# klkuhlm/unconfined

Measured on AMD Instinct MI355X. Metric: (t,r) drawdown points/sec, Neuman-1974 1024x256 sweep; max |rel err| vs CPU ref, higher is better.
Workload: dtype f64

## Files before the change

unconfined_amd/csrc/ucf_device.h:

```cpp

#include "ucf_math.h"
#include "ucf_plan.h"
#include <type_traits>

namespace UCF_NS {

using namespace ucfm;

#define UCF_STR_(x) #x
#define UCF_STR(x) UCF_STR_(x)
#define UCF_PI 3.14159265358979323846
#define UCF_EPS 2.220446049250313e-16

UCF_DEV double shfl_down1(double v) { return __shfl_down(v, 1, 64); }
UCF_DEV double shift_down1(double x)
{
    const int lo = __double2loint(x), hi = __double2hiint(x);
    const int l2 = __builtin_amdgcn_update_dpp(lo, lo, 0x130, 0xf, 0xf, false);
    const int h2 = __builtin_amdgcn_update_dpp(hi, hi, 0x130, 0xf, 0xf, false);
    return __hiloint2double(h2, l2);
}
UCF_DEV cplx shfl_down1(cplx v) { return cmake(shift_down1(v.re), shift_down1(v.im)); }
UCF_DEV cplx bcast0(cplx v) { return cmake(__shfl(v.re, 0, 64), __shfl(v.im, 0, 64)); }
UCF_DEV double wave_max(double v)
{
#pragma unroll
    for (int off = 32; off >= 1; off >>= 1) v = fmax(v, __shfl_xor(v, off, 64));
    return v;
}
UCF_DEV void stat_add(long long* ctr, bool pred)
{
    if (ctr == nullptr) return;
    unsigned long long bal = __ballot(pred);
    if (bal != 0ull && (threadIdx.x & 63) == 0) atomicAdd((unsigned long long*)ctr, (unsigned long long)__popcll(bal));
}

#ifndef UCF_TU
#define UCF_TU -1
#endif
#define UCF_TU_HAS(L) (UCF_TU < 0 || UCF_TU == (L))

typedef double2 lds_c;
UCF_DEV cplx lds_ld(const lds_c* base, int slot, int lane) { lds_c v = base[slot * UCF_WAVE + lane]; return cmake(v.x, v.y); }
UCF_DEV void lds_st(lds_c* base, int slot, int lane, cplx z) { base[slot * UCF_WAVE + lane] = make_double2(z.re, z.im); }
template <int PART = UCF_PART>
UCF_DEV cplx scr_ld(const lds_c* base, int slot, int lane) { lds_c v = base[slot * PART + (lane & (PART - 1))]; return cmake(v.x, v.y); }
template <int PART = UCF_PART>
UCF_DEV void scr_st(lds_c* base, int slot, int lane, cplx z) { base[slot * PART + (lane & (PART - 1))] = make_double2(z.re, z.im); }

#if UCF_FAST
UCF_DEV cplx cinv_plain_(cplx z)
{
    const double r = fast_rcp(z.re * z.re + z.im * z.im);
    return cmake(z.re * r, -(z.im * r));
}
#endif

UCF_DEV cplx lap_time(const ucf_dev_params& P, cplx p)
{
    if (P.timeType < 0) {
        const bool linear = P.timeType <= -101;
        const int n = linear ? -P.timeType - 100 : -P.timeType;
        cplx sum = cmake(0.0, 0.0);
        for (int k = 0; k < n; k++) {
            const cplx term = rscale(P.sched[n + k], cexp_(rscale(-P.sched[k], p)));
            sum = (k == 0) ? term : cadd(sum, term);
        }
        const cplx num = csub(sum, rscale(P.sched[2 * n + 1], cexp_(rscale(-P.sched[2 * n], p))));
        return cdiv(num, linear ? cmul(p, p) : p);
    }
    const double t1 = P.timePar[0], t2 = P.timePar[1];
    switch (P.timeType) {
    case 1: return cdiv(cexp_(cscale(p, -t1)), p);
    case 2: return csub(cdiv(cexp_(cscale(p, -t1)), p), cdiv(cexp_(cscale(p, -t2)), p));
    case 3: return cexp_(cscale(p, -t1));
    case 4: {
        cplx a = rdiv(1.0, csub(p, cmul(p, cexp_(cscale(p, -t1)))));
        cplx b = rsub(1.0, cexp_(cscale(p, -t2)));
        return cdiv(cmul(a, b), p);
    }
    case 5: return cdiv(cexp_(cscale(p, -t2)), cadd(p, cmul(p, cexp_(cscale(p, -t1)))));
    case 6: return cdiv(cmul(cexp_(cscale(p, -t2)), p), caddr(cmul(p, p), t1 * t1));
    case 7: return cmake(0.0, 0.0);
    case 8: {
        cplx ex = cexp_(cdivr(cscale(p, -t1), 2.0));
        cplx num = cmul(cexp_(cscale(p, -t2)), rsub(1.0, ex));
        return cdiv(num, cmul(radd(1.0, ex), p));
    }
    default: return cmake(__builtin_nan(""), __builtin_nan(""));
    }
}

struct k01 { cplx k0, k1; int ierr; };
UCF_DEV cplx clog_(cplx z) { return cmake(log(hypot(z.re, z.im)), atan2(z.im, z.re)); }

__device__ __noinline__ static k01 cbesk01_(cplx z)
{
    k01 out;
    out.k0 = cmake(0.0, 0.0); out.k1 = out.k0; out.ierr = 0;
    const double tol = UCF_EPS;
    const double elim = 2.303 * (1021.0 * log10(2.0) - 3.0);
    const double alim = elim + fmax(-(log10(2.0) * 52.0 * 2.303), -41.45);
    const double at1 = 0.78539816339744830962;
    const double pi = 4.0 * at1, hpi = 2.0 * at1, spi = 3.0 / (2.0 * at1);
    const double rthpi = sqrt(8.0 * at1) / 2.0, fpi = 1.89769999331517738, tth = 6.66666666666666666e-01;
    const double gamma_e = 5.77215664901532861e-01;
    const double xx = z.re, yy = z.im;
    if (xx == 0.0 && yy == 0.0) { out.ierr = 1; return out; }
    const double caz = hypot(xx, yy);
    if (caz > 1073741823.5) { out.ierr = 4; return out; }
    if (caz < UCF_DBL_MIN * 1.0e3) { out.ierr = 2; return out; }
    if (!(caz > tol) && -log(0.5 * caz) > elim) { out.ierr = 2; return out; }
    const cplx rz = cdiv(cmake(2.0, 0.0), z);
    cplx s1, s2;
    if (caz <= 2.0) {
        const cplx smu = clog_(rz);
        cplx f = cadd(rscale(-gamma_e, cmake(1.0, 0.0)), cscale(smu, 1.0));
        cplx p = cmake(0.5, 0.0), q = cmake(0.5, 0.0);
        s1 = f; s2 = p;
        double ak = 1.0, a1 = 1.0, bk = 1.0;
        cplx ck = cmake(1.0, 0.0);
        if (caz >= tol) {
            const cplx cz = cscale(cmul(z, z), 0.25);
            const double t1 = 0.25 * caz * caz;
            do {
// ... 1371 lines not shown
    const ucf_dev_params& P = P0;
    UCF_K1_ASSUME
#endif
    const int lane = threadIdx.x & (UCF_WAVE - 1), wv = __builtin_amdgcn_readfirstlane(threadIdx.x / UCF_WAVE);
    constexpr int EF = (FAMILY == 5) ? 1 : FAMILY;
    constexpr bool ZPAIR = FOLD && EF == 2 && NZC == 1;
    const int nz = NZC ? NZC : P0.nz, R = P0.R, nacc = P0.nacc, N = P0.N, ngl = P0.ngl;
    __builtin_assume(nz >= 1 && R >= 1 && nacc >= 1 && ngl >= 1);
    const int nabs = N + nacc * ngl;
    {
        const double2* __restrict__ gt = (const double2*)P0.sc_tab;
        for (int k = threadIdx.x; k < UCF_SC_ENTRIES; k += UCF_WAVE * UCF_IWPB) lds[k] = gt[k];
    }
    __syncthreads();
    const lds_c* sct = lds;
    const int lslots = (NZC ? R : R + 1) * nz;
    lds_c* const wlds = lds + UCF_SC_ENTRIES + (size_t)wv * lslots * UCF_WAVE;
    lds_c* accTS = wlds;
    lds_c* accCur = wlds + (size_t)R * nz * UCF_WAVE;
    int ustat = blockIdx.x * UCF_IWPB + wv - gridDim.x * UCF_IWPB;
    auto next_unit = [&]() {
        if (!wcount) return ustat += gridDim.x * UCF_IWPB;
        int u = 0;
        if (lane == 0) u = __hip_atomic_fetch_add(wcount, 1, __ATOMIC_RELAXED, __HIP_MEMORY_SCOPE_AGENT);
        return __builtin_amdgcn_readfirstlane(u);
    };
    for (int wi = next_unit(); wi < nworkw; wi = next_unit()) {
        const bool tail = wi >= nheadw;
        const int ls = tail ? (lsplit >> 8) : (lsplit & 255), nsplit = 1 << ls;
        const int wj = tail ? wi - nheadw : wi;
        const int pt = (tail ? (nheadw >> (lsplit & 255)) : 0) + (wj >> ls), sub = wj & (nsplit - 1);
        auto part_bound = [&](int k) {
            if (k <= 0) return 0;
            if (k >= nsplit) return nabs;
            int j = (k * nabs / nsplit - N + ngl / 2) / ngl;
            j = j < 0 ? 0 : (j > nacc ? nacc : j);
            return N + j * ngl;
        };
        const int n0 = part_bound(sub), n1 = part_bound(sub + 1);
        if (n1 <= n0 && sub != 0) continue;
#ifdef UCF_TIMELINE
        const unsigned long long tl_t0 = __builtin_amdgcn_s_memtime();
#endif
        const work_item W = decode_item<LAYOUT>(P0, pt, lane, per_point, nr, nt, ir0, npts);
        const ucf_dev_params& P = item_params<MULTI>(P0, Pv, (LAYOUT == 3 ? W.plan * ppp : W.pidx) + pbase, ppp);
        bool need_lay1 = false, need_lay3 = false, need_lay12 = false;
        for (int z = 0; z < nz; z++) { need_lay1 |= (P.zLay[z] == 1); need_lay3 |= (P.zLay[z] == 3); need_lay12 |= (P.zLay[z] != 3); }
        const double tD = tDv[W.it], rD = rDv[W.ir];
        const int sv = (LAYOUT == 1) ? svmin : svv[W.it];
        const double2* __restrict__ row = tab + (size_t)(per_point ? W.pidx : (W.ir * nsv + (sv - svmin))) * nabs;
        const double tee = 2.0 * tD;
        const double sigma = P.alpha - P.logtol / (2.0 * tee);
        const cplx p = cmake(sigma, UCF_PI * W.mlap / tee);
        const double2 ltv = ltab[(size_t)(W.mlap < P0.np ? W.mlap : P0.np - 1) * nrows + W.it];
        const cplx lt = cmake(ltv.x, ltv.y);
        const lane_consts LC = make_lane_consts(P, p, lt);
        auto lt_again = [&]() {
            int it = W.it;
            asm volatile("" : "+v"(it));
            const double2 v = ltab[(size_t)(W.mlap < P0.np ? W.mlap : P0.np - 1) * nrows + it];
            return cmake(v.x, v.y);
        };
        double2* __restrict__ sti = state + (size_t)pt * state_slots(P0) * UCF_WAVE;
        double2* __restrict__ areas = sti + (size_t)(R + 1) * nz * UCF_WAVE;
        for (int s = 0; s < lslots; s++) lds_st(wlds, s, lane, cmake(0.0, 0.0));
        fast_common F;
        sc_ctx_init(F.sc, sct, UCF_KV(FAMILY, FOLD));
        const bool lane_ok = FAMILY != 2 || (fabs(LC.xifac.re) + fabs(LC.xifac.im) < 1.0e90);
        const int nlim = (__builtin_amdgcn_ballot_w64(!lane_ok) == 0) ? n1 : n0;

        int n = n0;
        double2 aa = row[n0 < nabs ? n0 : 0];
        int m = 0, jj = n0 > N ? (n0 - N) / ngl : 0;
        cplx acc0 = cmake(0.0, 0.0), acc1 = cmake(0.0, 0.0);
        int zph = 0;
        if constexpr (ZPAIR) {
            int stopped = 0;
            zph = 0;
            static_assert(!ZPAIR || (LAYOUT == 1 && !MULTI),
                          "the interval ends and the limits of the bounds stand behind the rows of a grid's abscissa table only");
            const double* __restrict__ ends = (const double*)tab + abscissa_ends_offset((size_t)nr * nsv, nabs) + (size_t)(W.ir * nsv + (sv - svmin)) * (nacc + 1);
            const double* __restrict__ zb = (const double*)tab + abscissa_limits_offset((size_t)nr * nsv, nabs, nacc);
            int settled = 0;
            if (nlim > n0) zph = zpair_part_phase(P, LC, ends[nlim > N ? (nlim - N + ngl - 1) / ngl : 0]);
            const int nts = nlim < N ? nlim : N;
            auto proven_run = [&](auto cls, auto beta, int nend) {
                for (; n < nend; n++) {
                    const double2 nxt = row[n + 1 < nabs ? n + 1 : n];
                    F.sc.salt = n;
                    (void)fast_eta<2, true>(P, LC, aa.x, F);
                    const cplx val = rscale(aa.y, fast_sample_zpair_proven<decltype(cls)::value, decltype(beta)::value>(P, LC, F));
                    const int n1 = n + 1;
                    int tz = __builtin_ctz(n1);
                    if (tz > R - 1) tz = R - 1;
                    for (int sh = 0; sh <= tz; sh++) {
                        const int j = R - sh;
                        const double wl = P.ts_w[(size_t)(j - 1) * N + ((n1 >> sh) - 1)];
                        lds_st(accTS, j - 1, lane, cadd(lds_ld(accTS, j - 1, lane), rscale(wl, val)));
                    }
                    aa = nxt;
                }
            };
            auto proven_run_class = [&](auto cls, int nend) {
                if (P.beta != 0.0) proven_run(cls, std::true_type(), nend);
                else proven_run(cls, std::false_type(), nend);
            };
            constexpr int TS_RUNS = 2;
            for (int k = 1; k <= TS_RUNS && n < nts; k++) {
                int nend = k * N / TS_RUNS;
                if (nend > nts) nend = nts;
                if (nend <= n) continue;
                int cls = UCF_IV_EX_SHORT;
                if (!settled) {
                    int known;
                    cls = zpair_interval_class(P, LC, n == 0 ? 0.0 : aa.x, row[nend - 1].x, P.zD[0], &known, zb);
                    zph |= known;
                    if (cls == UCF_IV_EX_SHORT && (zph & UCF_PH_RANGE)) settled = 1;
                }
                if (cls == UCF_IV_CS_TAB) proven_run_class(std::integral_constant<int, UCF_IV_CS_TAB>(), nend);
                else if (cls == UCF_IV_CS_SHORT) proven_run_class(std::integral_constant<int, UCF_IV_CS_SHORT>(), nend);
                else if (cls == UCF_IV_EX_TAB) proven_run_class(std::integral_constant<int, UCF_IV_EX_TAB>(), nend);
                else if (cls == UCF_IV_EX_SHORT) proven_run_class(std::integral_constant<int, UCF_IV_EX_SHORT>(), nend);
                else {
                    for (; n < nend; n++) {
                        const double2 nxt = row[n + 1 < nabs ? n + 1 : n];
                        F.sc.salt = n;
                        if (!fast_eta_wave_zpair(P, LC, aa.x, F, zph, 1)) { stopped = 1; break; }
                        const cplx val = rscale(aa.y, fast_sample_zpair(P, LC, F, zph, 1));
                        const int n1 = n + 1;
                        int tz = __builtin_ctz(n1);
                        if (tz > R - 1) tz = R - 1;
                        for (int sh = 0; sh <= tz; sh++) {
                            const int j = R - sh;
                            const double wl = P.ts_w[(size_t)(j - 1) * N + ((n1 >> sh) - 1)];
                            lds_st(accTS, j - 1, lane, cadd(lds_ld(accTS, j - 1, lane), rscale(wl, val)));
                        }
                        aa = nxt;
                    }
                    if (stopped) break;
                }
                UCF_UNIFORM_BLOCK();
            }
            auto proven_interval = [&](auto cls, auto beta) {
                for (int i = 0; i < ngl; i++, n++) {
                    const double2 nxt = row[n + 1 < nabs ? n + 1 : n];
                    F.sc.salt = n;
                    (void)fast_eta<2, true>(P, LC, aa.x, F);
                    const cplx fz = fast_sample_zpair_proven<decltype(cls)::value, decltype(beta)::value>(P, LC, F);
                    acc0 = cmake(__builtin_fma(fz.re, aa.y, acc0.re), __builtin_fma(fz.im, aa.y, acc0.im));
                    aa = nxt;
                }
            };
            auto proven_class = [&](auto cls) {
                if (P.beta != 0.0) proven_interval(cls, std::true_type());
                else proven_interval(cls, std::false_type());
            };
            double lob_next = 0.0;
            if (!stopped && n < nlim) lob_next = ends[jj];
            if (!stopped) while (n < nlim) {
                const double lob = lob_next;
                const double hib = lob_next = ends[jj + 1];
                int cls = UCF_IV_UNPROVEN;
                if (settled) cls = UCF_IV_EX_SHORT;
                else {
                    int known;
                    cls = zpair_interval_class(P, LC, lob, hib, P.zD[0], &known, zb);
                    zph |= known;
                    if (cls == UCF_IV_EX_SHORT && (zph & UCF_PH_RANGE)) settled = 1;
                }
                if (cls == UCF_IV_CS_TAB) proven_class(std::integral_constant<int, UCF_IV_CS_TAB>());
                else if (cls == UCF_IV_CS_SHORT) proven_class(std::integral_constant<int, UCF_IV_CS_SHORT>());
                else if (cls == UCF_IV_EX_TAB) proven_class(std::integral_constant<int, UCF_IV_EX_TAB>());
                else if (cls == UCF_IV_EX_SHORT) proven_class(std::integral_constant<int, UCF_IV_EX_SHORT>());
                else {
                    for (m = 0; m < ngl; m++, n++) {
                        const double2 nxt = row[n + 1 < nabs ? n + 1 : n];
                        F.sc.salt = n;
                        const int last = m == ngl - 1;
                        if (!fast_eta_wave_zpair(P, LC, aa.x, F, zph, last)) { stopped = 1; break; }
                        const cplx fz = fast_sample_zpair(P, LC, F, zph, last);
                        acc0 = cmake(__builtin_fma(fz.re, aa.y, acc0.re), __builtin_fma(fz.im, aa.y, acc0.im));
                        aa = nxt;
                    }
                    if (stopped) break;
                }
                UCF_UNIFORM_BLOCK();
                {
                    const double hw = (hib - lob) / 2.0;
                    const cplx ar = cmul(rscale(hw, acc0), lt_again());
                    areas[(size_t)jj * UCF_WAVE + lane] = make_double2(ar.re, ar.im);
                    acc0 = cmake(0.0, 0.0);
                    m = 0;
                    jj++;
                }
            }
        } else
        for (; n < nlim; n++) {
            const double2 nxt = row[n + 1 < nabs ? n + 1 : n];
            const bool ts = n < N;
            F.sc.salt = n;
            if (!fast_eta_wave<EF>(P, LC, aa.x, F)) break;
            fast_common_terms<EF, FOLD, LAY3, LAY1, NOFOLD>(P, LC, aa.x, need_lay1, F, need_lay3, need_lay12);
            const int n1 = n + 1;
            int tz = __builtin_ctz(n1);
            if (tz > R - 1) tz = R - 1;
            for (int z = 0; z < nz; z++) {
                const cplx fz = fast_sample_z<EF, FOLD, LAY3, LAY1, NOFOLD>(P, F, z);
                if (ts) {
                    const cplx val = rscale(aa.y, fz);
                    for (int sh = 0; sh <= tz; sh++) {
                        const int j = R - sh;
                        const double wl = P.ts_w[(size_t)(j - 1) * N + ((n1 >> sh) - 1)];
                        const int slot = (j - 1) * nz + z;
                        lds_st(accTS, slot, lane, cadd(lds_ld(accTS, slot, lane), rscale(wl, val)));
                    }
                } else if (nz == 1 || (NZC == 2 && z == 0)) {
                    acc0 = cmake(__builtin_fma(fz.re, aa.y, acc0.re), __builtin_fma(fz.im, aa.y, acc0.im));
                } else if (NZC == 2) {
                    acc1 = cmake(__builtin_fma(fz.re, aa.y, acc1.re), __builtin_fma(fz.im, aa.y, acc1.im));
                } else {
                    const cplx a1 = lds_ld(accCur, z, lane);
                    lds_st(accCur, z, lane, cmake(__builtin_fma(fz.re, aa.y, a1.re), __builtin_fma(fz.im, aa.y, a1.im)));
                }
            }
            if (!ts && ++m == ngl) {
                const double lob = P.j0z[sv + jj - 1] / rD;
                const double hib = P.j0z[sv + jj] / rD;
                const double hw = (hib - lob) / 2.0;
                for (int z = 0; z < nz; z++) {
                    const cplx run = (nz == 1 || (NZC == 2 && z == 0)) ? acc0 : (NZC == 2 ? acc1 : lds_ld(accCur, z, lane));
                    const cplx ar = cmul(rscale(hw, run), lt);
                    areas[(size_t)(jj * nz + z) * UCF_WAVE + lane] = make_double2(ar.re, ar.im);
                    if (nz != 1 && NZC != 2) lds_st(accCur, z, lane, cmake(0.0, 0.0));
                }
                acc0 = acc1 = cmake(0.0, 0.0);
                m = 0;
                jj++;
            }
            aa = nxt;
        }
        if (sub == 0) {
            const cplx lte = ZPAIR ? lt_again() : lt;
            for (int s = 0; s < R * nz; s++) {
                const cplx v = cmul(lds_ld(wlds, s, lane), lte);
                sti[(size_t)s * UCF_WAVE + lane] = make_double2(v.re, v.im);
            }
            for (int s = R * nz; s < (R + 1) * nz; s++) sti[(size_t)s * UCF_WAVE + lane] = make_double2(0.0, 0.0);
        }
#ifdef UCF_TIMELINE
        if (sub == 0) {
            const unsigned long long tl_t1 = __builtin_amdgcn_s_memtime();
            const unsigned hwid = __builtin_amdgcn_s_getreg(63492);
            if (lane == 0) sti[(size_t)(R * nz) * UCF_WAVE + 0] = make_double2(__longlong_as_double((long long)tl_t0), __longlong_as_double((long long)tl_t1));
            if (lane == 1) sti[(size_t)(R * nz) * UCF_WAVE + 1] = make_double2((double)hwid, (double)__builtin_amdgcn_s_getreg(63508));
// ... 476 lines not shown
```

unconfined_amd/csrc/ucf_fastpath.h:

```cpp
#pragma once

namespace UCF_NS {

#define UCF_UNIFORM_BLOCK() asm volatile("" ::: "memory")
#define UCF_UNIFORM_BLOCK_F(FAMILY) do { if constexpr ((FAMILY) != 4) UCF_UNIFORM_BLOCK(); } while (0)

struct fprim {
    double ch, sh, ei, sn, cs;
};

template <bool POS, bool SMALLY = false>
UCF_DEV fprim prim_from_e(double x, double ax, double e, double ei, double y, const sc_ctx& sc)
{
    const int salt = sc.salt;
    fprim f;
    f.ei = ei;
    const double he = 0.5 * e;
    f.ch = __builtin_fma(0.5, ei, he);
    double s;
    if (ax < 0.35) {
        const double x2 = ax * ax;
        double pl = addk(mulk(x2, UCF_KHERE(1.0 / 6227020800.0, salt)), UCF_KHERE(1.0 / 39916800.0, salt));
        pl = fmak(pl, x2, UCF_KHERE(1.0 / 362880.0, salt));
        pl = fmak(pl, x2, UCF_KHERE(1.0 / 5040.0, salt));
        pl = fmak(pl, x2, UCF_KHERE(1.0 / 120.0, salt));
        pl = fmak(pl, x2, UCF_KHERE(1.0 / 6.0, salt));
        s = __builtin_fma(ax * x2, pl, ax);
    } else {
        s = __builtin_fma(-0.5, ei, he);
    }
    f.sh = POS ? s : copysign(s, x);
    if (SMALLY) sincos_small_(y, sc, &f.sn, &f.cs);
    else sincos_tab_(y, sc, &f.sn, &f.cs);
    return f;
}
template <bool POS = false>
UCF_DEV fprim prim(double x, double y, const sc_ctx& sc)
{
    const double ax = POS ? x : fabs(x);
    const double e = exp_tab_(ax, sc);
    return prim_from_e<POS>(x, ax, e, fast_rcp(e), y, sc);
}
UCF_DEV void prim_pair_min(double x, double y, double zD, double xcap, const sc_ctx& sc, fprim* f, fprim* fz)
{
    double xc;
    asm("v_min_f64 %0, %1, %2" : "=v"(xc) : "v"(x), "s"(xcap));
    const double xz = xc * zD;
    const double e = exp_tab_(xc, sc), ez = exp_tab_(xz, sc);
    const double r = fast_rcp(e * ez);
    *f = prim_from_e<true>(xc, xc, e, r * ez, y, sc);
    *fz = prim_from_e<true>(xz, xz, ez, r * e, y * zD, sc);
}
UCF_DEV fprim prim_difference(const fprim& a, const fprim& b)
{
    fprim f;
    const double e = (a.ch + a.sh) * b.ei;
    const double ei = a.ei * (b.ch + b.sh);
    f.ei = ei;
    f.ch = 0.5 * (e + ei);
    f.sh = 0.5 * (e - ei);
    f.sn = __builtin_fma(a.sn, b.cs, -(a.cs * b.sn));
    f.cs = __builtin_fma(a.cs, b.cs, a.sn * b.sn);
    return f;
}
UCF_DEV cplx pcosh(const fprim& f) { return cmake(f.ch * f.cs, f.sh * f.sn); }
UCF_DEV cplx psinh(const fprim& f) { return cmake(f.sh * f.cs, f.ch * f.sn); }
UCF_DEV cplx pexpneg(const fprim& f) { return cmake(f.ei * f.cs, -(f.ei * f.sn)); }

UCF_DEV cplx expneg_direct(double x, double y, const sc_ctx& sc)
{
    const double ei = exp_tab_(-x, sc);
    double sn, cs;
    sincos_tab_(y, sc, &sn, &cs);
    return cmake(ei * cs, -(ei * sn));
}

UCF_DEV cplx expneg_small(double x, double y, const sc_ctx& sc)
{
    const double ei = exp_tab_(-x, sc);
    double sn, cs;
    sincos_small_(y, sc, &sn, &cs);
    return cmake(ei * cs, -(ei * sn));
}
UCF_DEV void prim_pair_small(double x, double y, double zD, double xcap, const sc_ctx& sc, fprim* f, fprim* fz)
{
    double xc;
    asm("v_min_f64 %0, %1, %2" : "=v"(xc) : "v"(x), "s"(xcap));
    const double xz = xc * zD;
    const double e = exp_tab_(xc, sc), ez = exp_tab_(xz, sc);
    const double r = fast_rcp(e * ez);
    *f = prim_from_e<true, true>(xc, xc, e, r * ez, y, sc);
    *fz = prim_from_e<true, true>(xz, xz, ez, r * e, y * zD, sc);
}

UCF_DEV cplx cfma(cplx a, cplx b, cplx c)
{
    return cmake(__builtin_fma(a.re, b.re, __builtin_fma(-a.im, b.im, c.re)), __builtin_fma(a.re, b.im, __builtin_fma(a.im, b.re, c.im)));
}
UCF_DEV cplx cfnma(cplx a, cplx b, cplx c)
{
    return cmake(__builtin_fma(-a.re, b.re, __builtin_fma(a.im, b.im, c.re)), __builtin_fma(-a.re, b.im, __builtin_fma(-a.im, b.re, c.im)));
}
UCF_DEV cplx cinv_plain(cplx z)
{
    const double r = fast_rcp(z.re * z.re + z.im * z.im);
    return cmake(z.re * r, -(z.im * r));
}
UCF_DEV cplx cinv_scaled(cplx z)
{
    const double m = fmax(fabs(z.re), fabs(z.im));
    const int il = __builtin_amdgcn_frexp_exp(m) - 1;
    const double c = ldexp(z.re, -il), d = ldexp(z.im, -il);
    const double r = fast_rcp(c * c + d * d);
    return cmake(ldexp(c * r, -il), ldexp(-(d * r), -il));
}

UCF_DEV cplx cinv_auto(cplx z)
{
    const double m = fmax(fabs(z.re), fabs(z.im));
    if (__builtin_amdgcn_ballot_w64(!(m < 1.0e150 && m > 1.0e-150)) == 0) return cinv_plain(z);
    return cinv_scaled(z);
}

struct lane_consts {
    cplx p, lt, xifac;
    cplx fdB1;
    cplx mnpv;
};

UCF_DEV lane_consts make_lane_consts(const ucf_dev_params& P, cplx p, cplx lt)
{
    lane_consts L;
    L.p = p;
    L.lt = lt;
    cplx xf = rscale(P.alphaD, cinv_plain(p));
    if (P.model == 3) {
        cplx sum = cmake(0.0, 0.0);
        for (int j = 0; j < P.MoenchM; j++) sum = cadd(sum, cinv_plain(radd(1.0, cscale(p, P.MoenchInvGamma[j]))));
        xf = cmul(cscale(xf, (double)P.MoenchM), cinv_plain(sum));
    }
    L.xifac = xf;
    L.fdB1 = cscale(cscale(cscale(p, P.fd_beta0), P.fd_expmb2), P.inv_kappa);
    L.mnpv = radd(1.0, cscale(p, P.mn_vartheta * P.mn_c3));
    return L;
}

struct fast_common {
    sc_ctx sc;
    cplx th, eta, ff1, ff2, inv_she, she, che, top, g3, inv_den, ex1;
    fprim p1;
    int have_p1;
    cplx mn_uod;
    cplx fd_s1;
    cplx top3, fd_s13;
    bool small_eta, fd_use, fd_use3;
    int any_small, any_large;
};

template <int FAMILY>
UCF_DEV double fast_scale(const ucf_dev_params& P)
{
    if (FAMILY == 0 || FAMILY == 3) return 2.0;
    if (FAMILY == 5) return P.inv_bD;
    return (FAMILY == 2 && P.model == 4) ? 2.0 : 2.0 * P.inv_bD;
}

template <int FAMILY, bool PAIR = false>
UCF_DEV bool fast_eta(const ucf_dev_params& P, const lane_consts& L, double a, fast_common& S)
{
    const double a2 = a * a;
    const cplx q = caddr(L.p, a2);
    double mq = 0.0;
    if (PAIR && FAMILY != 0) {
        double r;
        rsq_pair(q.re * q.re + q.im * q.im, &mq, &r);
        S.th = cmake(q.re * r, -(q.im * r));
    } else {
        const double r = fast_rcp(q.re * q.re + q.im * q.im);
        S.th = cmake(q.re * r, -(q.im * r));
    }
    if (FAMILY == 0) return q.re > 0.0;
    if (PAIR) {
        const double qi = q.im * P.inv_kappa;
        double r, hr;
        sqrt_hrsqrt(__builtin_fma(q.re, P.half_inv_kappa, mq * P.half_inv_kappa), &r, &hr);
        S.eta = cmake(r, qi * hr);
    } else {
        const double qr = q.re * P.inv_kappa, qi = q.im * P.inv_kappa;
        double r, hr;
        const double d = sqrt_only(__builtin_fma(qr, qr, qi * qi));
        sqrt_hrsqrt(0.5 * (d + qr), &r, &hr);
        S.eta = cmake(r, qi * hr);
    }
    return (S.eta.re <= P.fast_eta_max) & (q.re > 0.0) & (fabs(S.eta.im) < P.fast_im_max);
}
template <int FAMILY, bool PAIR = false>
UCF_DEV bool fast_eta_wave(const ucf_dev_params& P, const lane_consts& L, double a, fast_common& S)
{
    (void)fast_eta<FAMILY, PAIR>(P, L, a, S);
    const cplx q = caddr(L.p, a * a);
    unsigned long long bad = __builtin_amdgcn_ballot_w64(!(q.re > 0.0));
    if (FAMILY != 0) {
        bad |= __builtin_amdgcn_ballot_w64(!(S.eta.re <= P.fast_eta_max));
        bad |= __builtin_amdgcn_ballot_w64(!(fabs(S.eta.im) < P.fast_im_max));
    }
    return bad == 0;
}

enum {
    UCF_PH_RANGE = 1,
    UCF_PH_IM = 2,
    UCF_PH_LARGE = 4,
    UCF_PH_YS = 8,
    UCF_PH_YL = 16
};
UCF_DEV int zpair_part_phase(const ucf_dev_params& P, const lane_consts& L, double a_max)
{
    const double lim = 0.99 * P.fast_eta_max;
    const bool ok = (L.p.re > 0.0) & (lim > 0.0) & ((__builtin_fma(a_max, a_max, fabs(L.p.re) + fabs(L.p.im)) * P.inv_kappa) < lim * lim);
    return __builtin_amdgcn_ballot_w64(!ok) == 0 ? UCF_PH_RANGE : 0;
}
UCF_DEV bool fast_eta_wave_zpair(const ucf_dev_params& P, const lane_consts& L, double a, fast_common& S, int& ph, int may_set)
{
    (void)fast_eta<2, true>(P, L, a, S);
    unsigned long long bad = 0;
    if (!(ph & UCF_PH_RANGE)) {
        const cplx q = caddr(L.p, a * a);
        bad |= __builtin_amdgcn_ballot_w64(!(q.re > 0.0));
        bad |= __builtin_amdgcn_ballot_w64(!(S.eta.re <= P.fast_eta_max));
        UCF_UNIFORM_BLOCK();
    }
    if (!(ph & UCF_PH_IM)) {
        const double ai = fabs(S.eta.im);
        bad |= __builtin_amdgcn_ballot_w64(!(ai < P.fast_im_max));
        if (may_set && __builtin_amdgcn_ballot_w64(!(ai < 0.5 * P.fast_im_max)) == 0) ph |= UCF_PH_IM;
        UCF_UNIFORM_BLOCK();
    }
    return bad == 0;
}

template <int FAMILY, bool FOLD = false, bool LAY3 = true, bool LAY1 = true, bool NOFOLD = false>
UCF_DEV void fast_common_terms(const ucf_dev_params& P, const lane_consts& L, double a, bool need_lay1_in, fast_common& S,
                               bool need_lay3_in = false, bool need_lay12 = true)
{
    const double a2 = a * a;
    if (FAMILY == 0) return;
    if (FAMILY == 3) {
        const fprim p1 = prim<true>(S.eta.re, S.eta.im, S.sc);
        S.che = pcosh(p1);
        S.she = psinh(p1);
        const double wr = __builtin_fma(a2, P.mn_c3, L.mnpv.re), wi = L.mnpv.im;
        double vr, hr;
        sqrt_hrsqrt(0.5 * (sqrt_only(__builtin_fma(wr, wr, wi * wi)) + wr), &vr, &hr);
        const cplx u = cmake(P.mn_u0 * (1.0 - vr), -(P.mn_u0 * (wi * hr)));
        const cplx Delta0 = cfnma(u, S.che, cmul(S.eta, S.she));
        S.mn_uod = cmul(u, cinv_auto(Delta0));
        return;
    }
    const bool hantush = NOFOLD || !(FAMILY == 2 && P.model == 4);
    const bool z1 = FOLD || (!NOFOLD && P.fold_dD != 0), z2 = FOLD || (!NOFOLD && P.fold_lD1 != 0);
    const bool need_lay1 = (FOLD || !LAY1) ? false : need_lay1_in;
    const bool need_lay3 = (FOLD || !LAY3) ? false : need_lay3_in;
    S.small_eta = (FAMILY != 2) || (S.eta.re < P.maxexp);
    S.any_small = ((FAMILY != 2) || (__builtin_amdgcn_ballot_w64(S.small_eta) != 0)) ? 1 : 0;
    S.any_large = ((FAMILY == 2) && (__builtin_amdgcn_ballot_w64(!S.small_eta) != 0)) ? 1 : 0;
    const bool need_p1 = (hantush && (!(z1 && z2) || need_lay1)) || FAMILY == 4 || (FAMILY == 2 && S.any_small);
    S.have_p1 = (need_p1 && !z2) ? 1 : 0;
    fprim p1;
    if (need_p1) {
        p1 = prim<true>(S.eta.re, S.eta.im, S.sc);
        if (!z2) S.p1 = p1;
        S.che = pcosh(p1);
        S.she = psinh(p1);
        if (need_lay1) S.ex1 = pexpneg(p1);
        else S.ex1 = cmake(0.0, 0.0);
    } else {
        S.che = S.she = S.ex1 = cmake(0.0, 0.0);
    }
    if (hantush) {
        fprim pd;
        if (!z1) { pd = prim<true>(S.eta.re * P.dD, S.eta.im * P.dD, S.sc); S.ff1 = psinh(pd); }
        else S.ff1 = cmake(0.0, 0.0);
        fprim pl;
        if (!z2) { pl = prim<true>(S.eta.re * P.lD1, S.eta.im * P.lD1, S.sc); S.ff2 = psinh(pl); }
        else S.ff2 = cmake(0.0, 0.0);
        if (!(z1 && z2) || need_lay1) S.inv_she = cinv_auto(S.she);
        if (need_lay1) {
            const cplx exl = z2 ? cmake(1.0, 0.0) : pexpneg(pl);
            S.g3 = csub(exl, cmul(cadd(S.ff1, cmul(S.ex1, S.ff2)), S.inv_she));
        }
        if (FAMILY != 1) {
            S.top = S.top3 = S.th;
            if (!(z1 && z2)) {
                if (need_lay12) {
                    cplx g1;
                    if (z1) g1 = cmake(1.0, 0.0);
                    else if (P.share_g1top == 1) g1 = pcosh(pd);
// ... 72 lines not shown
{
    const bool z1 = FOLD || (!NOFOLD && P.fold_dD != 0), z2 = FOLD || (!NOFOLD && P.fold_lD1 != 0);
    const int lay = (FOLD || (!LAY1 && lay_in == 1)) ? 2 : lay_in;
    const bool need_chz = (lay == 1) || !z1 || (FAMILY == 2 && S.any_small) || FAMILY == 4;
    cplx chz = cmake(1.0, 0.0);
    fprim pz;
    if (need_chz) { pz = prim<true>(S.eta.re * zD, S.eta.im * zD, S.sc); chz = pcosh(pz); }
    *chz_out = chz;
    cplx udp;
    if (lay == 1) {
        udp = cmul(S.g3, chz);
    } else {
        cplx g2 = cmake(0.0, 0.0);
        const bool need_1z = !z2;
        fprim p1z;
        if (z2 && FAMILY == 2 && S.any_large) {
            const double c = 1.0 - zD;
            *exz_out = expneg_direct(S.eta.re * c, S.eta.im * c, S.sc);
            UCF_UNIFORM_BLOCK_F(FAMILY);
        }
        if (need_1z) {
            if (need_chz && S.have_p1 && zD >= 0.0 && zD <= 1.0) p1z = prim_difference(S.p1, pz);
            else
            { const double c = 1.0 - zD; p1z = prim(S.eta.re * c, S.eta.im * c, S.sc); }
        }
        if (!z2 && FAMILY == 2 && S.any_large) { *exz_out = pexpneg(p1z); UCF_UNIFORM_BLOCK_F(FAMILY); }
        cplx f2c = cmake(0.0, 0.0);
        if (!z2) f2c = cmul(S.ff2, pcosh(p1z));
        if (lay == 2 || !LAY3) {
            if (z1 && z2) { UCF_UNIFORM_BLOCK_F(FAMILY); return S.th; }
            cplx num = f2c;
            if (!z1) { num = cadd(cmul(S.ff1, chz), f2c); UCF_UNIFORM_BLOCK_F(FAMILY); }
            g2 = cmul(num, S.inv_she);
            udp = rsub(1.0, g2);
            UCF_UNIFORM_BLOCK_F(FAMILY);
        } else {
            const double ca = 2.0 - zD - P.dD, cb = zD - P.dD;
            const cplx sa = psinh(prim(S.eta.re * ca, S.eta.im * ca, S.sc));
            const cplx sb = psinh(prim(S.eta.re * cb, S.eta.im * cb, S.sc));
            const cplx num = cmake(__builtin_fma(0.5, sa.re + sb.re, -f2c.re), __builtin_fma(0.5, sa.im + sb.im, -f2c.im));
            udp = cmul(num, S.inv_she);
        }
    }
    const cplx res = cmul(udp, S.th);
    UCF_UNIFORM_BLOCK_F(FAMILY);
    return res;
}

template <int FAMILY, bool FOLD = false, bool LAY3 = true, bool LAY1 = true, bool NOFOLD = false>
UCF_DEV cplx fast_sample_z(const ucf_dev_params& P, const fast_common& S, int iz)
{
    const double zD = P.zD[iz];
    const int lay = P.zLay[iz];
    cplx chz, exz = cmake(0.0, 0.0);
    if (FAMILY == 0) return S.th;
    if (FAMILY == 3) {
        const cplx cz = pcosh(prim<true>(S.eta.re * zD, S.eta.im * zD, S.sc));
        return cfma(S.th, cmul(S.mn_uod, cz), S.th);
    }
    if (FAMILY == 1) return fast_hantush_z<1, FOLD, LAY3, LAY1, NOFOLD>(P, S, zD, lay, &chz, &exz);
    if (FAMILY == 4) {
        const cplx sH = fast_hantush_z<4, FOLD, LAY3, LAY1, NOFOLD>(P, S, zD, lay, &chz, &exz);
        if (!FOLD && LAY3 && lay == 3) return S.fd_use3 ? cadd(sH, cmul(S.fd_s13, chz)) : sH;
        return S.fd_use ? cadd(sH, cmul(S.fd_s1, chz)) : sH;
    }
    cplx u;
    if (!NOFOLD && P.model == 4) {
        u = S.th;
        if (S.any_small) chz = pcosh(prim(S.eta.re * zD, S.eta.im * zD, S.sc));
        if (S.any_large) { const double c = 1.0 - zD; exz = expneg_direct(S.eta.re * c, S.eta.im * c, S.sc); }
    } else {
        u = fast_hantush_z<2, FOLD, LAY3, LAY1, NOFOLD>(P, S, zD, lay, &chz, &exz);
        if (LAY1 && S.any_large && lay == 1) { const double c = 1.0 - zD; exz = expneg_direct(S.eta.re * c, S.eta.im * c, S.sc); }
    }
    const cplx top = (!FOLD && LAY3 && (NOFOLD || P.model != 4) && lay == 3) ? S.top3 : S.top;
    cplx g = chz;
    if (S.any_large) {
        g = S.small_eta ? chz : exz;
        asm volatile("" ::: "memory");
    }
    return cfnma(cmul(top, g), S.inv_den, u);
}

template <bool SMALLY, int KB = -1>
UCF_DEV void zpair_arm_small(const ucf_dev_params& P, const lane_consts& L, const fast_common& S, double zD, cplx* g, cplx* den)
{
    fprim p1, pz;
    if (SMALLY) prim_pair_small(S.eta.re, S.eta.im, zD, P.maxexp, S.sc, &p1, &pz);
    else prim_pair_min(S.eta.re, S.eta.im, zD, P.maxexp, S.sc, &p1, &pz);
    *g = pcosh(pz);
    const cplx che = pcosh(p1), she = psinh(p1);
    const cplx xi = cmul(S.eta, L.xifac);
    if (KB < 0 ? P.beta != 0.0 : KB != 0) *den = cfma(radd(1.0, cmul(rscale(P.beta, S.eta), xi)), che, cmul(xi, she));
    else *den = cfma(xi, she, che);
}
template <bool SMALLY, int KB = -1>
UCF_DEV void zpair_arm_large(const ucf_dev_params& P, const lane_consts& L, const fast_common& S, double x, double y, cplx* g, cplx* den)
{
    *g = SMALLY ? expneg_small(x, y, S.sc) : expneg_direct(x, y, S.sc);
    const cplx xi = cmul(S.eta, L.xifac);
    if (KB < 0 ? P.beta != 0.0 : KB != 0) *den = cadd(radd(1.0, cmul(rscale(P.beta, S.eta), xi)), xi);
    else *den = radd(1.0, xi);
}
UCF_DEV cplx fast_sample_zpair(const ucf_dev_params& P, const lane_consts& L, const fast_common& S, int& ph, int may_set)
{
    const double zD = P.zD[0];
    int form = 2;
    if (!(ph & UCF_PH_LARGE)) {
        const bool small_eta = S.eta.re < P.maxexp;
        const bool any_small = __builtin_amdgcn_ballot_w64(small_eta) != 0, any_large = __builtin_amdgcn_ballot_w64(!small_eta) != 0;
        form = !any_large ? 0 : (any_small ? 1 : 2);
        double mx = P.maxexp;
        asm volatile("" : "+s"(mx));
        if (may_set && form == 2 && __builtin_amdgcn_ballot_w64(!(S.eta.re > mx * (1.0 + 0x1p-20))) == 0) ph |= UCF_PH_LARGE;
        UCF_UNIFORM_BLOCK();
    }
    cplx den, g;
    if (form == 0) {
        if (may_set && !(ph & UCF_PH_YS)) {
            if (__builtin_amdgcn_ballot_w64(!(fabs(S.eta.im) < UCF_SC_SMALL)) == 0) ph |= UCF_PH_YS | UCF_PH_YL;
            UCF_UNIFORM_BLOCK();
        }
        if (ph & UCF_PH_YS) {
            zpair_arm_small<true>(P, L, S, zD, &g, &den);
            UCF_UNIFORM_BLOCK();
        } else {
            zpair_arm_small<false>(P, L, S, zD, &g, &den);
            UCF_UNIFORM_BLOCK();
        }
    } else if (form == 2) {
        const double c = 1.0 - zD;
        const double x = S.eta.re * c, y = S.eta.im * c;
        if (may_set && !(ph & UCF_PH_YL)) {
            if (__builtin_amdgcn_ballot_w64(!(fabs(y) < UCF_SC_SMALL)) == 0) ph |= UCF_PH_YL;
            UCF_UNIFORM_BLOCK();
        }
        if (ph & UCF_PH_YL) {
            zpair_arm_large<true>(P, L, S, x, y, &g, &den);
            UCF_UNIFORM_BLOCK();
        } else {
            zpair_arm_large<false>(P, L, S, x, y, &g, &den);
            UCF_UNIFORM_BLOCK();
        }
    } else {
        const bool small_eta = S.eta.re < P.maxexp;
        fprim p1, pz;
        prim_pair_min(S.eta.re, S.eta.im, zD, P.maxexp, S.sc, &p1, &pz);
        const cplx chz = pcosh(pz), che = pcosh(p1), she = psinh(p1);
        const cplx xi = cmul(S.eta, L.xifac);
        if (P.beta != 0.0) {
            const cplx one_bex = radd(1.0, cmul(rscale(P.beta, S.eta), xi));
            den = small_eta ? cfma(one_bex, che, cmul(xi, she)) : cadd(one_bex, xi);
        } else {
            den = small_eta ? cfma(xi, she, che) : radd(1.0, xi);
        }
        const double c = 1.0 - zD;
        const cplx exz = expneg_direct(S.eta.re * c, S.eta.im * c, S.sc);
        g = small_eta ? chz : exz;
        UCF_UNIFORM_BLOCK();
    }
    const double r = fast_rcp(__builtin_fma(den.im, den.im, den.re * den.re));
    const cplx inv_den = cmake(den.re * r, -(den.im * r));
    return cfnma(cmul(S.th, g), inv_den, S.th);
}

enum {
    UCF_IV_UNPROVEN = 0,
    UCF_IV_CS_TAB = 1,
    UCF_IV_CS_SHORT = 2,
    UCF_IV_EX_TAB = 3,
    UCF_IV_EX_SHORT = 4
};
static_assert(UCF_ZB_SC_SMALL == UCF_SC_SMALL, "the plan's short sin/cos limit (ucf_launch_plan.h) is sincos_small_'s");
UCF_DEV int zpair_unit_bounds(const double* __restrict__ zb, const lane_consts& L, double lob, double hib, int* ph_proven)
{
    *ph_proven = 0;
    const double u = __builtin_fma(fabs(L.p.im), 0.5, L.p.re), i2 = L.p.im * L.p.im;
    const double up_hi = __builtin_fma(hib, hib, u);
    const double lo_lo = __builtin_fma(lob, lob, L.p.re);
    const bool in_range = (L.p.re > 0.0) & (up_hi < zb[UCF_ZB_RANGE]) & (i2 < zb[UCF_ZB_IM] * lo_lo);
    if (__builtin_amdgcn_ballot_w64(!in_range) != 0) return -1;
    const bool ys = __builtin_amdgcn_ballot_w64(!(i2 < zb[UCF_ZB_YS] * lo_lo)) == 0;
    if (__builtin_amdgcn_ballot_w64(!(up_hi < zb[UCF_ZB_CS])) == 0) {
        if (ys) { *ph_proven = UCF_PH_IM | UCF_PH_YS | UCF_PH_YL; return UCF_IV_CS_SHORT; }
        if (__builtin_amdgcn_ballot_w64(i2 >= zb[UCF_ZB_YS] * __builtin_fma(lob, lob, u)) == 0) return -1;
        *ph_proven = UCF_PH_IM;
        return UCF_IV_CS_TAB;
    }
    if (__builtin_amdgcn_ballot_w64(!(lo_lo > zb[UCF_ZB_EX])) == 0) {
        if (ys || __builtin_amdgcn_ballot_w64(!(i2 < zb[UCF_ZB_YL] * lo_lo)) == 0) {
            *ph_proven = UCF_PH_IM | UCF_PH_LARGE | UCF_PH_YL | (ys ? UCF_PH_YS : 0);
            return UCF_IV_EX_SHORT;
        }
        if (__builtin_amdgcn_ballot_w64(i2 >= zb[UCF_ZB_YL] * __builtin_fma(lob, lob, u)) == 0) return -1;
        *ph_proven = UCF_PH_IM | UCF_PH_LARGE;
        return UCF_IV_EX_TAB;
    }
    return -1;
}
UCF_DEV int zpair_interval_class(const ucf_dev_params& P, const lane_consts& L, double lob, double hib, double zD, int* ph_proven,
                                 const double* __restrict__ zb)
{
    if (const int c = zpair_unit_bounds(zb, L, lob, hib, ph_proven); c >= 0) return c;
    UCF_UNIFORM_BLOCK();
    *ph_proven = 0;
    fast_common T;
    (void)fast_eta<2, true>(P, L, hib, T);
    const double re_hi = T.eta.re;
    (void)fast_eta<2, true>(P, L, lob, T);
    const double re_lo = T.eta.re, im_lo = fabs(T.eta.im);
    const bool in_range = (L.p.re > 0.0) & (re_hi * 1.01 <= P.fast_eta_max) & (im_lo * 2.0 < P.fast_im_max);
    if (__builtin_amdgcn_ballot_w64(!in_range) != 0) return UCF_IV_UNPROVEN;
    *ph_proven = UCF_PH_IM;
    const bool ys = __builtin_amdgcn_ballot_w64(!(im_lo < UCF_SC_SMALL)) == 0;
    const bool yl = ys || __builtin_amdgcn_ballot_w64(!(im_lo * (1.0 - zD) < UCF_SC_SMALL)) == 0;
    if (ys) *ph_proven |= UCF_PH_YS;
    if (yl) *ph_proven |= UCF_PH_YL;
    if (__builtin_amdgcn_ballot_w64(!(re_hi * (1.0 + 0x1p-20) < P.maxexp)) == 0) return ys ? UCF_IV_CS_SHORT : UCF_IV_CS_TAB;
    if (__builtin_amdgcn_ballot_w64(!(re_lo * (1.0 - 0x1p-20) > P.maxexp)) == 0) {
        *ph_proven |= UCF_PH_LARGE;
        return yl ? UCF_IV_EX_SHORT : UCF_IV_EX_TAB;
    }
    return UCF_IV_UNPROVEN;
}
template <int CLS, bool BETA>
UCF_DEV cplx fast_sample_zpair_proven(const ucf_dev_params& P, const lane_consts& L, const fast_common& S)
{
    const double zD = P.zD[0];
    cplx den, g;
    if (CLS == UCF_IV_CS_TAB || CLS == UCF_IV_CS_SHORT) {
        zpair_arm_small<CLS == UCF_IV_CS_SHORT, BETA ? 1 : 0>(P, L, S, zD, &g, &den);
    } else {
        const double c = 1.0 - zD;
        const double x = S.eta.re * c, y = S.eta.im * c;
        zpair_arm_large<CLS == UCF_IV_EX_SHORT, BETA ? 1 : 0>(P, L, S, x, y, &g, &den);
    }
    const double r = fast_rcp(__builtin_fma(den.im, den.im, den.re * den.re));
    const cplx inv_den = cmake(den.re * r, -(den.im * r));
    return cfnma(cmul(S.th, g), inv_den, S.th);
}


}
```

unconfined_amd/csrc/ucf_launch_plan.h:

```cpp
#pragma once
#include "../../include/ucf.h"
#include "ucf_env.h"

#define UCF_WAVE 64
#define UCF_MAX_R 16
#define UCF_LDS_C 16

struct ucf_dev_params {
    int model, MNtype, order, timeType, MoenchM;
    int M, np, k, N, R, nacc, ngl, nz;
    int tab_premul;
    int nj0z, any_lay3;
    int any_lay1;
    int any_fold;
    int nz_out, z_off;
    double timePar[2];
    double kappa, alphaD, beta;
    double lD, dD, bD, dD1, lD1;
    double MoenchInvGamma[UCF_MAX_MOENCH];
    double alpha, logtol, maxexp;
    double inv_kappa, inv_bD, fast_eta_max, fast_im_max;
    int fold_dD, fold_lD1, share_g1top, _pad2;
    double g1_delta;
    double hs_rDw, hs_CDw, hs_tDb;
    double mn_vartheta, mn_u0, mn_c3;
    double fd_h, fd_invhsq, fd_beta0, fd_beta3, fd_expmb2;
    double fd_isk, fd_gmax;
    double hv[UCF_MAX_R];
    double zD[UCF_MAX_NZ];
    int zLay[UCF_MAX_NZ];
    const double* ts_x;
    const double* ts_w;
    const double* gl_x;
    const double* gl_w;
    const double* j0z;
    const double* fd_e;
    const double* sched;
    const double* sc_tab;
    double half_inv_kappa;
};
#define UCF_ZB_SC_SMALL 0.012
enum { UCF_ZB_RANGE = 0, UCF_ZB_IM, UCF_ZB_CS, UCF_ZB_EX, UCF_ZB_YS, UCF_ZB_YL, UCF_ZB_COUNT = 8 };
static constexpr double zpair_bound_limit(const ucf_dev_params& dp, int which)
{
    const double lim = 0.99 * dp.fast_eta_max, me2 = dp.kappa * (dp.maxexp * dp.maxexp), c = 1.0 - dp.zD[0];
    const double ys = 4.0 * dp.kappa * (UCF_ZB_SC_SMALL * UCF_ZB_SC_SMALL);
    switch (which) {
    case UCF_ZB_RANGE: return lim > 0.0 ? dp.kappa * (lim * lim) : 0.0;
    case UCF_ZB_IM: return dp.kappa * (dp.fast_im_max * dp.fast_im_max);
    case UCF_ZB_CS: return me2 / (1.0 + 0x1p-19);
    case UCF_ZB_EX: return me2 / (1.0 - 0x1p-19);
    case UCF_ZB_YS: return ys;
    case UCF_ZB_YL: return ys / (c * c);
    default: return 0.0;
    }
}
static constexpr size_t abscissa_ends_offset(size_t nrows, size_t nabs) { return nrows * nabs * 2; }
static constexpr size_t abscissa_limits_offset(size_t nrows, size_t nabs, size_t nacc) { return nrows * (nabs * 2 + nacc + 1); }
static constexpr size_t abscissa_table_doubles(size_t nrows, size_t nabs, size_t nacc) { return abscissa_limits_offset(nrows, nabs, nacc) + UCF_ZB_COUNT; }
#define UCF_SC_ENTRIES (256 + 128)
#define UCF_IWPB 4

#define UCF_PART 16
#define UCF_WYNN_REGS 12

#ifndef UCF_FOLD_WAVES
#define UCF_FOLD_WAVES 5
#endif
#ifndef UCF_UNFOLD_WAVES
#define UCF_UNFOLD_WAVES 4
#endif
#ifndef UCF_TAIL_LSPLIT_DEFAULT
#define UCF_TAIL_LSPLIT_DEFAULT 3
#endif
#ifndef UCF_NZC
#define UCF_NZC(F, FO) (LAYOUT == 1 && (F) == 2 && (FO) ? 1 : 0)
#endif
#ifndef UCF_NZC2
#define UCF_NZC2(F, FO) ((LAYOUT == 1 || LAYOUT == 3) ? 2 : 0)
#endif

static inline int family_of(const ucf_dev_params& dp)
{
    switch (dp.model) {
    case 0: return 0;
    case 1: return 1;
    case 2: return 5;
    case 3: case 4: case 5: return 2;
    case 6: return dp.MNtype == 1 ? 3 : (dp.MNtype == 2 ? 4 : -1);
    default: return -1;
    }
}

static inline bool areas_in_lds(const ucf_dev_params& dp)
{
    const size_t with_areas = ((size_t)(dp.R + 1 + dp.nacc) * dp.nz * UCF_WAVE + (size_t)(2 * dp.nacc > dp.R ? 2 * dp.nacc : dp.R) * UCF_PART) * UCF_LDS_C;
    return with_areas <= 20 * 1024;
}

static inline size_t point_lds_bytes(const ucf_dev_params& dp, bool fast, bool resume = false)
{
    size_t bytes = ((size_t)(dp.R + 1 + ((areas_in_lds(dp) && !resume) ? dp.nacc : 0)) * dp.nz * UCF_WAVE + (size_t)(2 * dp.nacc > dp.R ? 2 * dp.nacc : dp.R) * UCF_PART) * UCF_LDS_C;
    if (!fast && family_of(dp) == 4) bytes += 2 * (size_t)dp.order * UCF_WAVE * UCF_LDS_C;
    return bytes;
}

static inline size_t samples_lds_bytes(const ucf_dev_params& dp, bool fast)
{
    if (fast) return UCF_SC_ENTRIES * UCF_LDS_C;
    return family_of(dp) == 4 ? 2 * (size_t)dp.order * UCF_WAVE * UCF_LDS_C : 16;
}

static inline int split_kind(const ucf_dev_params& dp, bool fast)
{
    const int fam = family_of(dp);
    if (fast) {
        if (fam >= 0 && fam <= 5) return 1;
    } else if (fam == 4 && 2 * (size_t)dp.order * UCF_WAVE * UCF_LDS_C > 16 * 1024) return 0;
    return 2;
}

struct ucf_transform_buffers {
    size_t ndone, todo, defer, wcount;
    size_t ints;
    size_t state_item_bytes;
    size_t ltab;
    size_t state_bytes;
};
static inline ucf_transform_buffers transform_buffers(const ucf_dev_params& dp, bool fast, size_t nwork, size_t lt_rows)
{
    const int kind = split_kind(dp, fast);
    ucf_transform_buffers b;
    b.ndone = 0;
    b.todo = b.ndone + nwork;
    b.defer = b.todo + 1 + nwork;
    b.wcount = b.defer + 1 + nwork * (size_t)dp.nz;
// ... 128 lines not shown
```

Baseline: 9.811 million.

## Add proven sinh-no-series interval classes and drop clamp in proven cosh arms

Adds a new phase bit and bound entry that prove, per interval, that the real part of eta times zD exceeds the sinh series threshold, so the proven cosh/sinh sample path can use specialized classes that skip the small-argument sinh polynomial branch. The proven small arms also skip the v_min clamp against maxexp, since the interval class already proves the bound. The time-stepping weights load is additionally routed through the constant address space to encourage scalar loads. This adds more template instantiations, which raises code size and register pressure risk.

```diff
diff --git a/unconfined_amd/csrc/ucf_device.h b/unconfined_amd/csrc/ucf_device.h
--- a/unconfined_amd/csrc/ucf_device.h
+++ b/unconfined_amd/csrc/ucf_device.h
@@ -41,6 +41,7 @@
 #define UCF_TU_HAS(L) (UCF_TU < 0 || UCF_TU == (L))
 
 typedef double2 lds_c;
+typedef __attribute__((address_space(4))) double ucf_const_double;
 UCF_DEV cplx lds_ld(const lds_c* base, int slot, int lane) { lds_c v = base[slot * UCF_WAVE + lane]; return cmake(v.x, v.y); }
 UCF_DEV void lds_st(lds_c* base, int slot, int lane, cplx z) { base[slot * UCF_WAVE + lane] = make_double2(z.re, z.im); }
 template <int PART = UCF_PART>
@@ -1578,6 +1579,7 @@
             const double* __restrict__ ends = (const double*)tab + abscissa_ends_offset((size_t)nr * nsv, nabs) + (size_t)(W.ir * nsv + (sv - svmin)) * (nacc + 1);
             const double* __restrict__ zb = (const double*)tab + abscissa_limits_offset((size_t)nr * nsv, nabs, nacc);
             int settled = 0;
+            const ucf_const_double* const tsw = (const ucf_const_double*)P.ts_w;
             if (nlim > n0) zph = zpair_part_phase(P, LC, ends[nlim > N ? (nlim - N + ngl - 1) / ngl : 0]);
             const int nts = nlim < N ? nlim : N;
             auto proven_run = [&](auto cls, auto beta, int nend) {
@@ -1591,7 +1593,7 @@
                     if (tz > R - 1) tz = R - 1;
                     for (int sh = 0; sh <= tz; sh++) {
                         const int j = R - sh;
-                        const double wl = P.ts_w[(size_t)(j - 1) * N + ((n1 >> sh) - 1)];
+                        const double wl = tsw[(size_t)(j - 1) * N + ((n1 >> sh) - 1)];
                         lds_st(accTS, j - 1, lane, cadd(lds_ld(accTS, j - 1, lane), rscale(wl, val)));
                     }
                     aa = nxt;
@@ -1628,7 +1630,7 @@
                         if (tz > R - 1) tz = R - 1;
                         for (int sh = 0; sh <= tz; sh++) {
                             const int j = R - sh;
-                            const double wl = P.ts_w[(size_t)(j - 1) * N + ((n1 >> sh) - 1)];
+                            const double wl = tsw[(size_t)(j - 1) * N + ((n1 >> sh) - 1)];
                             lds_st(accTS, j - 1, lane, cadd(lds_ld(accTS, j - 1, lane), rscale(wl, val)));
                         }
                         aa = nxt;
@@ -1664,8 +1666,11 @@
                     zph |= known;
                     if (cls == UCF_IV_EX_SHORT && (zph & UCF_PH_RANGE)) settled = 1;
                 }
+                if ((zph & UCF_PH_SH) && (cls == UCF_IV_CS_TAB || cls == UCF_IV_CS_SHORT)) cls += UCF_IV_CS_TAB_SH - UCF_IV_CS_TAB;
                 if (cls == UCF_IV_CS_TAB) proven_class(std::integral_constant<int, UCF_IV_CS_TAB>());
                 else if (cls == UCF_IV_CS_SHORT) proven_class(std::integral_constant<int, UCF_IV_CS_SHORT>());
+                else if (cls == UCF_IV_CS_TAB_SH) proven_class(std::integral_constant<int, UCF_IV_CS_TAB_SH>());
+                else if (cls == UCF_IV_CS_SHORT_SH) proven_class(std::integral_constant<int, UCF_IV_CS_SHORT_SH>());
                 else if (cls == UCF_IV_EX_TAB) proven_class(std::integral_constant<int, UCF_IV_EX_TAB>());
                 else if (cls == UCF_IV_EX_SHORT) proven_class(std::integral_constant<int, UCF_IV_EX_SHORT>());
                 else {
diff --git a/unconfined_amd/csrc/ucf_fastpath.h b/unconfined_amd/csrc/ucf_fastpath.h
--- a/unconfined_amd/csrc/ucf_fastpath.h
+++ b/unconfined_amd/csrc/ucf_fastpath.h
@@ -9,7 +9,7 @@
     double ch, sh, ei, sn, cs;
 };
 
-template <bool POS, bool SMALLY = false>
+template <bool POS, bool SMALLY = false, bool NOSERIES = false>
 UCF_DEV fprim prim_from_e(double x, double ax, double e, double ei, double y, const sc_ctx& sc)
 {
     const int salt = sc.salt;
@@ -18,7 +18,9 @@
     const double he = 0.5 * e;
     f.ch = __builtin_fma(0.5, ei, he);
     double s;
-    if (ax < 0.35) {
+    if (NOSERIES) {
+        s = __builtin_fma(-0.5, ei, he);
+    } else if (ax < UCF_ZB_SINH_SERIES) {
         const double x2 = ax * ax;
         double pl = addk(mulk(x2, UCF_KHERE(1.0 / 6227020800.0, salt)), UCF_KHERE(1.0 / 39916800.0, salt));
         pl = fmak(pl, x2, UCF_KHERE(1.0 / 362880.0, salt));
@@ -41,15 +43,16 @@
     const double e = exp_tab_(ax, sc);
     return prim_from_e<POS>(x, ax, e, fast_rcp(e), y, sc);
 }
+template <bool CLAMP = true, bool NOSERIES = false>
 UCF_DEV void prim_pair_min(double x, double y, double zD, double xcap, const sc_ctx& sc, fprim* f, fprim* fz)
 {
-    double xc;
-    asm("v_min_f64 %0, %1, %2" : "=v"(xc) : "v"(x), "s"(xcap));
+    double xc = x;
+    if (CLAMP) asm("v_min_f64 %0, %1, %2" : "=v"(xc) : "v"(x), "s"(xcap));
     const double xz = xc * zD;
     const double e = exp_tab_(xc, sc), ez = exp_tab_(xz, sc);
     const double r = fast_rcp(e * ez);
-    *f = prim_from_e<true>(xc, xc, e, r * ez, y, sc);
-    *fz = prim_from_e<true>(xz, xz, ez, r * e, y * zD, sc);
+    *f = prim_from_e<true, false, NOSERIES>(xc, xc, e, r * ez, y, sc);
+    *fz = prim_from_e<true, false, NOSERIES>(xz, xz, ez, r * e, y * zD, sc);
 }
 UCF_DEV fprim prim_difference(const fprim& a, const fprim& b)
 {
@@ -82,15 +85,16 @@
     sincos_small_(y, sc, &sn, &cs);
     return cmake(ei * cs, -(ei * sn));
 }
+template <bool CLAMP = true, bool NOSERIES = false>
 UCF_DEV void prim_pair_small(double x, double y, double zD, double xcap, const sc_ctx& sc, fprim* f, fprim* fz)
 {
-    double xc;
-    asm("v_min_f64 %0, %1, %2" : "=v"(xc) : "v"(x), "s"(xcap));
+    double xc = x;
+    if (CLAMP) asm("v_min_f64 %0, %1, %2" : "=v"(xc) : "v"(x), "s"(xcap));
     const double xz = xc * zD;
     const double e = exp_tab_(xc, sc), ez = exp_tab_(xz, sc);
     const double r = fast_rcp(e * ez);
-    *f = prim_from_e<true, true>(xc, xc, e, r * ez, y, sc);
-    *fz = prim_from_e<true, true>(xz, xz, ez, r * e, y * zD, sc);
+    *f = prim_from_e<true, true, NOSERIES>(xc, xc, e, r * ez, y, sc);
+    *fz = prim_from_e<true, true, NOSERIES>(xz, xz, ez, r * e, y * zD, sc);
 }
 
 UCF_DEV cplx cfma(cplx a, cplx b, cplx c)
@@ -212,7 +216,8 @@
     UCF_PH_IM = 2,
     UCF_PH_LARGE = 4,
     UCF_PH_YS = 8,
-    UCF_PH_YL = 16
+    UCF_PH_YL = 16,
+    UCF_PH_SH = 32
 };
 UCF_DEV int zpair_part_phase(const ucf_dev_params& P, const lane_consts& L, double a_max)
 {
@@ -451,12 +456,12 @@
     return cfnma(cmul(top, g), S.inv_den, u);
 }
 
-template <bool SMALLY, int KB = -1>
+template <bool SMALLY, int KB = -1, bool PROVEN = false, bool SH = false>
 UCF_DEV void zpair_arm_small(const ucf_dev_params& P, const lane_consts& L, const fast_common& S, double zD, cplx* g, cplx* den)
 {
     fprim p1, pz;
-    if (SMALLY) prim_pair_small(S.eta.re, S.eta.im, zD, P.maxexp, S.sc, &p1, &pz);
-    else prim_pair_min(S.eta.re, S.eta.im, zD, P.maxexp, S.sc, &p1, &pz);
+    if (SMALLY) prim_pair_small<!PROVEN, SH>(S.eta.re, S.eta.im, zD, P.maxexp, S.sc, &p1, &pz);
+    else prim_pair_min<!PROVEN, SH>(S.eta.re, S.eta.im, zD, P.maxexp, S.sc, &p1, &pz);
     *g = pcosh(pz);
     const cplx che = pcosh(p1), she = psinh(p1);
     const cplx xi = cmul(S.eta, L.xifac);
@@ -538,8 +543,11 @@
     UCF_IV_CS_TAB = 1,
     UCF_IV_CS_SHORT = 2,
     UCF_IV_EX_TAB = 3,
-    UCF_IV_EX_SHORT = 4
+    UCF_IV_EX_SHORT = 4,
+    UCF_IV_CS_TAB_SH = 5,
+    UCF_IV_CS_SHORT_SH = 6
 };
+static_assert(UCF_IV_CS_SHORT_SH - UCF_IV_CS_SHORT == UCF_IV_CS_TAB_SH - UCF_IV_CS_TAB, "one offset takes a cosh/sinh class to its settled-sinh twin");
 static_assert(UCF_ZB_SC_SMALL == UCF_SC_SMALL, "the plan's short sin/cos limit (ucf_launch_plan.h) is sincos_small_'s");
 UCF_DEV int zpair_unit_bounds(const double* __restrict__ zb, const lane_consts& L, double lob, double hib, int* ph_proven)
 {
@@ -551,9 +559,10 @@
     if (__builtin_amdgcn_ballot_w64(!in_range) != 0) return -1;
     const bool ys = __builtin_amdgcn_ballot_w64(!(i2 < zb[UCF_ZB_YS] * lo_lo)) == 0;
     if (__builtin_amdgcn_ballot_w64(!(up_hi < zb[UCF_ZB_CS])) == 0) {
-        if (ys) { *ph_proven = UCF_PH_IM | UCF_PH_YS | UCF_PH_YL; return UCF_IV_CS_SHORT; }
+        const int sh = __builtin_amdgcn_ballot_w64(!(lo_lo > zb[UCF_ZB_SH])) == 0 ? UCF_PH_SH : 0;
+        if (ys) { *ph_proven = UCF_PH_IM | UCF_PH_YS | UCF_PH_YL | sh; return UCF_IV_CS_SHORT; }
         if (__builtin_amdgcn_ballot_w64(i2 >= zb[UCF_ZB_YS] * __builtin_fma(lob, lob, u)) == 0) return -1;
-        *ph_proven = UCF_PH_IM;
+        *ph_proven = UCF_PH_IM | sh;
         return UCF_IV_CS_TAB;
     }
     if (__builtin_amdgcn_ballot_w64(!(lo_lo > zb[UCF_ZB_EX])) == 0) {
@@ -585,7 +594,10 @@
     const bool yl = ys || __builtin_amdgcn_ballot_w64(!(im_lo * (1.0 - zD) < UCF_SC_SMALL)) == 0;
     if (ys) *ph_proven |= UCF_PH_YS;
     if (yl) *ph_proven |= UCF_PH_YL;
-    if (__builtin_amdgcn_ballot_w64(!(re_hi * (1.0 + 0x1p-20) < P.maxexp)) == 0) return ys ? UCF_IV_CS_SHORT : UCF_IV_CS_TAB;
+    if (__builtin_amdgcn_ballot_w64(!(re_hi * (1.0 + 0x1p-20) < P.maxexp)) == 0) {
+        if (__builtin_amdgcn_ballot_w64(!(re_lo * (1.0 - 0x1p-20) * zD >= UCF_ZB_SINH_SERIES)) == 0) *ph_proven |= UCF_PH_SH;
+        return ys ? UCF_IV_CS_SHORT : UCF_IV_CS_TAB;
+    }
     if (__builtin_amdgcn_ballot_w64(!(re_lo * (1.0 - 0x1p-20) > P.maxexp)) == 0) {
         *ph_proven |= UCF_PH_LARGE;
         return yl ? UCF_IV_EX_SHORT : UCF_IV_EX_TAB;
@@ -597,8 +609,9 @@
 {
     const double zD = P.zD[0];
     cplx den, g;
-    if (CLS == UCF_IV_CS_TAB || CLS == UCF_IV_CS_SHORT) {
-        zpair_arm_small<CLS == UCF_IV_CS_SHORT, BETA ? 1 : 0>(P, L, S, zD, &g, &den);
+    if (CLS != UCF_IV_EX_TAB && CLS != UCF_IV_EX_SHORT) {
+        constexpr bool SH = CLS == UCF_IV_CS_TAB_SH || CLS == UCF_IV_CS_SHORT_SH;
+        zpair_arm_small<CLS == UCF_IV_CS_SHORT || CLS == UCF_IV_CS_SHORT_SH, BETA ? 1 : 0, true, SH>(P, L, S, zD, &g, &den);
     } else {
         const double c = 1.0 - zD;
         const double x = S.eta.re * c, y = S.eta.im * c;
diff --git a/unconfined_amd/csrc/ucf_launch_plan.h b/unconfined_amd/csrc/ucf_launch_plan.h
--- a/unconfined_amd/csrc/ucf_launch_plan.h
+++ b/unconfined_amd/csrc/ucf_launch_plan.h
@@ -40,11 +40,13 @@
     double half_inv_kappa;
 };
 #define UCF_ZB_SC_SMALL 0.012
-enum { UCF_ZB_RANGE = 0, UCF_ZB_IM, UCF_ZB_CS, UCF_ZB_EX, UCF_ZB_YS, UCF_ZB_YL, UCF_ZB_COUNT = 8 };
+#define UCF_ZB_SINH_SERIES 0.35
+enum { UCF_ZB_RANGE = 0, UCF_ZB_IM, UCF_ZB_CS, UCF_ZB_EX, UCF_ZB_YS, UCF_ZB_YL, UCF_ZB_SH, UCF_ZB_COUNT = 8 };
 static constexpr double zpair_bound_limit(const ucf_dev_params& dp, int which)
 {
     const double lim = 0.99 * dp.fast_eta_max, me2 = dp.kappa * (dp.maxexp * dp.maxexp), c = 1.0 - dp.zD[0];
     const double ys = 4.0 * dp.kappa * (UCF_ZB_SC_SMALL * UCF_ZB_SC_SMALL);
+    const double sh = UCF_ZB_SINH_SERIES / dp.zD[0];
     switch (which) {
     case UCF_ZB_RANGE: return lim > 0.0 ? dp.kappa * (lim * lim) : 0.0;
     case UCF_ZB_IM: return dp.kappa * (dp.fast_im_max * dp.fast_im_max);
@@ -52,6 +54,7 @@
     case UCF_ZB_EX: return me2 / (1.0 - 0x1p-19);
     case UCF_ZB_YS: return ys;
     case UCF_ZB_YL: return ys / (c * c);
+    case UCF_ZB_SH: return dp.kappa * (sh * sh) / (1.0 - 0x1p-19);
     default: return 0.0;
     }
 }
```

Measured after the change: 9.920 million, median of 6. +1.1%, better.
